# byronknoll/cmix

Hardware: AMD Instinct MI355X
Metric: input bytes/s on enwik8 at 1 GPU; compressed-size parity vs CPU ref (higher is better)
Workload: dtype f32

## Files before the change

### cmix_amd/csrc/cmx_api.hip

```cpp
#include <hip/hip_runtime.h>
#include <math.h>
#include <stdio.h>
#include <stdlib.h>
#include <string.h>
#include <stddef.h>
#include <string>
#include <map>
#include <mutex>
#include <vector>

#include "../../include/cmix_amd.h"
#include "mixnet_state.h"
#include "cmx_late.h"
#include "cmx_streams.h"
#include "cmx_verify.h"

extern "C" __global__ void cmx_mixnet_kernel(MixState*, const float*, const uint32_t*,
                                             const uint8_t*, const float*, int, float*, float*, int);
extern "C" __global__ void cmx_mixnet_spec_kernel(MixState*, SpecXfer*, const float*, const uint32_t*, const uint8_t*, const float*, int, float*,
                                                  float*, int);
extern "C" __global__ void cmx_mixnet_spec_jitter_kernel(MixState*, SpecXfer*, const float*, const uint32_t*, const uint8_t*, const float*, int, float*, float*, int);
extern "C" __global__ void cmx_mixnet_spec_late_kernel(MixState*, SpecXfer*, const float*, const uint32_t*, const float*, int, float*, float*, int, CmxLate);
extern "C" __global__ void cmx_mixnet_spec_verify_kernel(MixState*, SpecXfer*, const float*, const uint32_t*, const uint8_t*, const float*, int, float*, float*, int,
                                                         CmxVerify);
// ... 243 lines not shown
  ALLOC(map_keys, uint32_t, (size_t)CMX_MIXERS * CMX_MAP_SLOTS, true);
  ALLOC(map_vals, uint32_t, (size_t)CMX_MIXERS * CMX_MAP_SLOTS, true);
  ALLOC(s6, uint16_t, (size_t)CMX_SM6_VOL * 8, false);
  ALLOC(s7, uint16_t, (size_t)CMX_SM7_VOL * 8, false);
  ALLOC(x1, int, CMX_MIX1_VOL, false);
  ALLOC(x2, int, CMX_MIX2_VOL, false);
#undef ALLOC
  for (int i = 0; i <= CMX_MIXERS; ++i) S.max_steps[i] = 1;
  S.steps = 0;
  S.sse_j = 1;
  S.sse_pc = 0;
  S.sse_ffl = 0;
  for (int i = 0; i <= CMX_MIXERS; ++i) S.fwd_p[i] = 0.5f;
  h->d_state = (MixState*)dalloc(sizeof(MixState), false);
  if (!h->d_state) { set_err("hipMalloc failed for state"); cmx_mixnet_destroy(h); return nullptr; }
  hipMemcpy(h->d_state, &S, sizeof S, hipMemcpyHostToDevice);
  hipLaunchKernelGGL(cmx_sse_init_kernel, dim3(2048), dim3(256), 0, 0, h->d_state);
  h->d_sync_probs = (float*)dalloc(CMX_IN0 * 4, true);
  h->d_sync_sel = (uint32_t*)dalloc(CMX_MIXERS * 4, true);
  h->d_sync_bit = (uint8_t*)dalloc(16, true);
  h->d_sync_p = (float*)dalloc(16, true);
  if (hipFuncSetAttribute((const void*)cmx_mixnet_kernel, hipFuncAttributeMaxDynamicSharedMemorySize,
                          (int)kLdsBytes) != hipSuccess) {
    set_err("hipFuncSetAttribute(MaxDynamicSharedMemorySize) failed");
    cmx_mixnet_destroy(h);
    return nullptr;
  }
  h->d_xfer = (SpecXfer*)dalloc(sizeof(SpecXfer), true);
  bool attr_ok = true;
  for (const void* k : {(const void*)cmx_mixnet_spec_kernel, (const void*)cmx_mixnet_spec_jitter_kernel, (const void*)cmx_mixnet_spec_late_kernel,
                        (const void*)cmx_mixnet_spec_verify_kernel})
    attr_ok = attr_ok && hipFuncSetAttribute(k, hipFuncAttributeMaxDynamicSharedMemorySize, CMX_SPEC_LDS_BYTES) == hipSuccess;
  if (!h->d_xfer || !attr_ok) {
    set_err("cmx_mixnet_create: hand-off area / kernel attribute (spec kernel) failed");
    cmx_mixnet_destroy(h);
    return nullptr;
  }
  { const char* v = getenv("CMX_MIXNET_DBG"); h->dbg = v ? atoi(v) : 0; }
  { const char* v = getenv("CMX_MIXNET_JITTER"); h->jitter = v ? atoi(v) & 15 : 0; }
  { const char* v = getenv("CMX_MIXNET_ROTATE"); h->rotate = v && v[0] == '1'; }
  { const char* v = getenv("CMX_MIXNET_XCD"); h->xcd = v ? atoi(v) : CMX_MIXNET_XCD_DEFAULT; if (h->xcd > 7) h->xcd = -1; }
  hipEventCreate(&h->ev0);
  hipEventCreate(&h->ev1);
  for (int i = 0; i < CMX_PIPELINE_SLOTS; ++i) { hipEventCreateWithFlags(&h->ev_decay[i], hipEventDisableTiming); hipEventCreateWithFlags(&h->ev_kdone[i], hipEventDisableTiming); }
  hipError_t e = hipDeviceSynchronize();
  if (e != hipSuccess) { set_err(std::string("init: ") + hipGetErrorString(e)); cmx_mixnet_destroy(h); return nullptr; }
  return h;
}

static inline float decay_of(uint64_t steps) {
  return (float)(0.9 / pow(0.0000001 * steps + 0.8, 0.8));
}

static int ensure_decay(cmx_mixnet_t* h, size_t nbits) {
  const int fail_value = 1;
  if (nbits <= h->decay_cap) return 0;
  size_t cap = nbits < 4096 ? 4096 : nbits;
  if (h->h_decay) hipHostFree(h->h_decay);
  h->h_decay = nullptr;
  for (int i = 0; i < CMX_PIPELINE_SLOTS; ++i) {
    if (h->decay_used[i]) { (void)hipEventSynchronize(h->ev_decay[i]); (void)hipEventSynchronize(h->ev_kdone[i]); }
    h->decay_used[i] = false;
  }
  HIP_OK(hipHostMalloc((void**)&h->h_decay, (size_t)CMX_PIPELINE_SLOTS * cap * 4, hipHostMallocDefault));
  void* p = nullptr;
  HIP_OK(hipMalloc(&p, (size_t)CMX_PIPELINE_SLOTS * cap * 4));
  h->allocs.push_back(p);
  h->d_decay = (float*)p;
  h->decay_cap = cap;
  return 0;
}

int cmx_mixnet_spec_stats(cmx_mixnet_t* h, uint64_t out[5]) {
  const int fail_value = 1;
  if (!h || !out) { set_err("cmx_mixnet_spec_stats: bad argument"); return 1; }
  HIP_OK(hipSetDevice(h->device));
  HIP_OK(hipDeviceSynchronize());
  unsigned long long st[8];
  HIP_OK(hipMemcpy(st, (char*)h->d_xfer + offsetof(SpecXfer, stat), sizeof st, hipMemcpyDeviceToHost));
  for (int i = 0; i < 5; ++i) out[i] = st[i];
  return 0;
}

static bool g_cumask_applied = false;
static bool cumask_wanted() {
  static const char* const xe = getenv("CMX_MIXNET_XCD");
  static const bool w = getenv("CMX_CUMASK") != nullptr && xe && atoi(xe) >= 0 && atoi(xe) < 8 && getenv("CMX_PIPELINE_STREAMS") == nullptr;
  return w;
}
namespace {
std::mutex g_q_mu;
std::map<hipStream_t, int> g_q_dev;
int g_q_held[64];
}
int cmx_make_stream(hipStream_t* st, int which) {
  *st = nullptr;
  int dev = 0, cus = 0;
  if (hipGetDevice(&dev) != hipSuccess || hipDeviceGetAttribute(&cus, hipDeviceAttributeMultiprocessorCount, dev) != hipSuccess || cus <= 0 || cus > 32 * 32) {
    set_err("cmx_make_stream: no device"); return 1;
  }
  std::lock_guard<std::mutex> g(g_q_mu);
  int& held = g_q_held[dev & 63];
  if (held + 1 > CMX_MAX_HW_QUEUES) {
    set_err("cmx_make_stream: this process already holds " + std::to_string(held) + " dedicated hardware queues on device " + std::to_string(dev) + ", the limit is " +
            std::to_string(CMX_MAX_HW_QUEUES) + " (an engine takes 13, 14 when it decodes; CMX_PIPELINE_STREAMS=2 or 1 takes 8 or 6)");
    return 1;
  }
  const int words = (cus + 31) / 32;
  std::vector<uint32_t> full(words, 0u);
  for (int cu = 0; cu < cus; ++cu) full[cu / 32] |= 1u << (cu % 32);
  hipError_t e = hipErrorUnknown;
  if (cumask_wanted() && which != 2) {
    static const int x = atoi(getenv("CMX_MIXNET_XCD"));
    std::vector<uint32_t> m(words, 0u);
    for (int cu = 0; cu < cus; ++cu) if (((cu & 7) == x) == (which == 1)) m[cu / 32] |= 1u << (cu % 32);
    e = hipExtStreamCreateWithCUMask(st, (uint32_t)words, m.data());
    if (e == hipSuccess) { if (which == 1) g_cumask_applied = true; }
    else (void)hipGetLastError();
  }
  if (e != hipSuccess) e = hipExtStreamCreateWithCUMask(st, (uint32_t)words, full.data());
  if (e != hipSuccess) { *st = nullptr; set_err(std::string("cmx_make_stream: hipExtStreamCreateWithCUMask: ") + hipGetErrorString(e)); return 1; }
  g_q_dev[*st] = dev;
  ++held;
  return 0;
}
void cmx_destroy_stream(hipStream_t st) {
  if (!st) return;
  {
    std::lock_guard<std::mutex> g(g_q_mu);
    auto it = g_q_dev.find(st);
    if (it != g_q_dev.end()) { --g_q_held[it->second & 63]; g_q_dev.erase(it); }
  }
  (void)hipStreamDestroy(st);
}
int cmx_hw_queues(int device) {
  std::lock_guard<std::mutex> g(g_q_mu);
  return g_q_held[device & 63];
}

__global__ void cmx_overlap_probe_kernel(unsigned* cnt, unsigned* seen, int i, unsigned n, unsigned long long ticks) {
  if (threadIdx.x != 0) return;
  __hip_atomic_fetch_add(cnt, 1u, __ATOMIC_RELAXED, __HIP_MEMORY_SCOPE_AGENT);
  const unsigned long long t0 = wall_clock64();
  unsigned c = __hip_atomic_load(cnt, __ATOMIC_RELAXED, __HIP_MEMORY_SCOPE_AGENT);
  while (c < n && wall_clock64() - t0 < ticks) { __builtin_amdgcn_s_sleep(8); c = __hip_atomic_load(cnt, __ATOMIC_RELAXED, __HIP_MEMORY_SCOPE_AGENT); }
  __hip_atomic_store(seen + i, c, __ATOMIC_RELAXED, __HIP_MEMORY_SCOPE_AGENT);
}
int cmx_overlap_probe(const hipStream_t* st, int n, int* distinct) {
  std::vector<hipStream_t> q;
  for (int i = 0; i < n; ++i) {
    if (!st[i]) continue;
    bool dup = false;
    for (hipStream_t s : q) dup = dup || s == st[i];
    if (!dup) q.push_back(st[i]);
  }
  if (distinct) *distinct = (int)q.size();
  if (q.empty()) return 0;
  int dev = 0, khz = 0;
  if (hipGetDevice(&dev) != hipSuccess || hipDeviceGetAttribute(&khz, hipDeviceAttributeWallClockRate, dev) != hipSuccess || khz <= 0) { set_err("cmx_overlap_probe: no device"); return -1; }
  const int m = (int)q.size();
  unsigned* d = nullptr;
  if (hipMalloc((void**)&d, (size_t)(1 + m) * 4) != hipSuccess) { set_err("cmx_overlap_probe: hipMalloc failed"); return -1; }
  bool ok = hipMemsetAsync(d, 0, (size_t)(1 + m) * 4, q[0]) == hipSuccess && hipStreamSynchronize(q[0]) == hipSuccess;
  const unsigned long long ticks = 50ull * (unsigned long long)khz;
  for (int i = 0; ok && i < m; ++i) {
    hipLaunchKernelGGL(cmx_overlap_probe_kernel, dim3(1), dim3(64), 0, q[i], d, d + 1, i, (unsigned)m, ticks);
// ... 429 lines not shown
```

### cmix_amd/csrc/mixnet_chunk.hip

```cpp
#include "mixnet_dev.h"
#include "cmx_late.h"
#include "cmx_verify.h"

namespace {

constexpr int SEG = 548;
constexpr unsigned SPIN_LIMIT = 1u << 27;

struct Ctl {
  int staged[2];
  int consumed;
  int u_epoch;
  int scout_epoch;
  int tail_in;
  int tail_done;
  int abort;
  int b_in, b_done;
  int bit_epoch;
  unsigned late_lo, late_hi;
};

struct BitRec {
  uint32_t rowidx[48];
  uint32_t changed[32];
// ... 46 lines not shown
}

__device__ __forceinline__ unsigned long long wave_sum_u64(unsigned long long v) {
#pragma unroll
  for (int o = 32; o > 0; o >>= 1) v += __shfl_xor(v, o, 64);
  return v;
}
__device__ __forceinline__ void verify_flag(const CmxVerify& V, unsigned long long key) {
  atomicAdd(&V.hdr->launch_count, 1ull);
  atomicMax(&V.hdr->launch_first, ~key);
}

typedef __attribute__((address_space(3))) int lds_int;
__device__ __forceinline__ int lds_poll(const int* p) {
  int v;
  asm volatile("ds_read_b32 %0, %1\n\ts_waitcnt lgkmcnt(0)" : "=v"(v) : "v"((const lds_int*)p) : "memory");
  return v;
}
__device__ __forceinline__ void lds_publish_store(int* p, int v) {
  asm volatile("s_waitcnt lgkmcnt(0)\n\tds_write_b32 %0, %1" :: "v"((lds_int*)p), "v"(v) : "memory");
}
__device__ __forceinline__ void touch_line(gptr<const float> g, unsigned lds_dst) {
  unsigned keep;
  const unsigned dst = __builtin_amdgcn_readfirstlane(lds_dst);
  asm volatile("s_mov_b32 %0, m0\n\ts_mov_b32 m0, %2\n\ts_nop 0\n\tglobal_load_lds_dword %1, off\n\ts_mov_b32 m0, %0"
               : "=&s"(keep) : "v"(g), "s"(dst) : "memory");
}
__device__ __forceinline__ void st_rel(int* p, int v) { lds_publish_store(p, v); }
__device__ __forceinline__ CmxLateBox* ctl_box(Ctl* ctl) {
  const unsigned lo = (unsigned)lds_poll((const int*)&ctl->late_lo), hi = (unsigned)lds_poll((const int*)&ctl->late_hi);
  return reinterpret_cast<CmxLateBox*>(((unsigned long long)hi << 32) | lo);
}
__device__ __forceinline__ bool late_expired(CmxLateBox* B, unsigned long long& t0) {
  if (late_ld(&B->abort) || late_ld(&B->fail)) return true;
  const unsigned long long now = wall_clock64();
  if (!t0) { t0 = now; return false; }
  if (now - t0 > late_timeout_ticks(B)) { late_st(&B->fail, 1u); return true; }
  return false;
}
template <bool LATE = false> __device__ __forceinline__ bool wait_ge(Ctl* ctl, const int* p, int target, bool sleepy) {
  unsigned spins = 0;
  unsigned long long t0 = 0;
  while (lds_poll(p) < target) {
    if (sleepy) __builtin_amdgcn_s_sleep(2);
    if ((++spins & 1023u) == 0) {
      bool out;
      if (LATE) { CmxLateBox* const B = ctl_box(ctl); out = B ? late_expired(B, t0) : spins > SPIN_LIMIT; }
      else out = spins > SPIN_LIMIT;
      if (lds_poll(&ctl->abort) || out) {
        lds_publish_store(&ctl->abort, 1);
        return false;
      }
    }
  }
  return true;
}

__device__ __forceinline__ float bcast_lane(float v, int j) {
  return __int_as_float(__builtin_amdgcn_readlane(__float_as_int(v), j));
}

__device__ __forceinline__ float clamp_med3(float x, float mn, float mx) { return __builtin_amdgcn_fmed3f(x, mn, mx); }
__device__ __forceinline__ float clamp_out(float x, float mn, float mx) {
  const float lo = x < mn ? mn : x;
  return x > mx ? mx : lo;
}

__device__ __forceinline__ float4 f4sub_mul(float4 w, float u, float4 x) {
  w.x = fsub(w.x, fmul(u, x.x));
  w.y = fsub(w.y, fmul(u, x.y));
  w.z = fsub(w.z, fmul(u, x.z));
  w.w = fsub(w.w, fmul(u, x.w));
  return w;
}
__device__ __forceinline__ float4 f4scale(float4 w, float c) {
  w.x = fmul(w.x, c); w.y = fmul(w.y, c); w.z = fmul(w.z, c); w.w = fmul(w.w, c);
  return w;
}
__device__ __forceinline__ float add4(float p, float4 v) {
  p = fadd(p, v.x); p = fadd(p, v.y); p = fadd(p, v.z); p = fadd(p, v.w);
  return p;
}

template <int NB> __device__ __forceinline__ float chain_seg_n(const float* rowp, int n, float p) {
  const float4* row = reinterpret_cast<const float4*>(__builtin_assume_aligned(rowp, 16));
  float4 a[8], b[8];
#pragma unroll
  for (int i = 0; i < 8; ++i) a[i] = row[i];
#pragma unroll 1
  for (int bi = 0; bi < NB; bi += 2) {
    __builtin_amdgcn_sched_barrier(0);
#pragma unroll
    for (int i = 0; i < 8; ++i) b[i] = row[(bi + 1) * 8 + i];
    __builtin_amdgcn_sched_barrier(0);
#pragma unroll
    for (int i = 0; i < 8; ++i) p = add4(p, a[i]);
    __builtin_amdgcn_sched_barrier(0);
#pragma unroll
    for (int i = 0; i < 8; ++i) a[i] = row[(bi + 2) * 8 + i];
    __builtin_amdgcn_sched_barrier(0);
#pragma unroll
    for (int i = 0; i < 8; ++i) p = add4(p, b[i]);
  }
  __builtin_amdgcn_sched_barrier(0);
  const int rem4 = (n >> 2) - NB * 8;
#pragma unroll
  for (int i = 0; i < 7; ++i)
    if (i < rem4) p = add4(p, a[i]);
  if (n & 2) {
    p = fadd(p, a[7].x);
    p = fadd(p, a[7].y);
  }
  return p;
}

struct U16x8 { unsigned w0, w1, w2, w3; };
__device__ __forceinline__ U16x8 load_cell(const uint16_t* p) {
  typedef unsigned v4u __attribute__((ext_vector_type(4)));
  v4u v = *(gptr<const v4u>)as_global(p);
  U16x8 r; r.w0 = v.x; r.w1 = v.y; r.w2 = v.z; r.w3 = v.w;
  return r;
}
__device__ __forceinline__ void store_cell_async(uint16_t* p, const U16x8& c) {
  typedef unsigned v4u __attribute__((ext_vector_type(4)));
  v4u o = {c.w0, c.w1, c.w2, c.w3};
  asm volatile("global_store_dwordx4 %0, %1, off\n\ts_nop 1" :: "v"(as_global(p)), "v"(o) : "memory");
}
__device__ __forceinline__ int cell_get(const U16x8& c, int i) {
  unsigned w = i < 2 ? c.w0 : i < 4 ? c.w1 : i < 6 ? c.w2 : c.w3;
  return (int)((i & 1) ? (w >> 16) : (w & 0xffffu));
}
__device__ __forceinline__ void cell_set(U16x8& c, int i, int v) {
  const unsigned m = (i & 1) ? 0x0000ffffu : 0xffff0000u, x = ((unsigned)v & 0xffffu) << ((i & 1) * 16);
  const int q = i >> 1;
  c.w0 = q == 0 ? (c.w0 & m) | x : c.w0;
  c.w1 = q == 1 ? (c.w1 & m) | x : c.w1;
  c.w2 = q == 2 ? (c.w2 & m) | x : c.w2;
  c.w3 = q == 3 ? (c.w3 & m) | x : c.w3;
}
__device__ __forceinline__ unsigned bcast_u(unsigned v) { return (unsigned)__builtin_amdgcn_readlane((int)v, 0); }

struct SseInterp {
  int freq, sw, P;
  __device__ __forceinline__ int pred(const U16x8& c, int iP) {
    freq = (6 * iP) >> 15;
    sw = (6 * iP) & 32767;
    int f = (((32768 - sw) * cell_get(c, freq) + sw * cell_get(c, freq + 1)) >> 15) - 8192;
    if (f <= 0) f = 1;
    if (f >= 32768) f = 32767;
    P = f;
    return f;
  }
  __device__ __forceinline__ void update(U16x8& c, int bit, int wr0) {
    P = (P * (32768 - wr0)) >> 15;
    if (bit == 0) P += wr0;
    const int c0 = cell_get(c, freq), c1 = cell_get(c, freq + 1);
    const int dC = c0 - c1;
    const int sw_dC = (sw * dC + 32767) >> 15;
    cell_set(c, freq, (uint16_t)(P + sw_dC + 8192));
    cell_set(c, freq + 1, (uint16_t)(P - (dC - sw_dC) + 8192));
  }
};

template <bool LATE, bool JIT = false, bool VER = false> __device__ void tail_a_role(MixState* S, const Lds& L, const float* decay1, int nbits, float* mix_out, int lane, bool prof_on,
                                                                     const CmxVerify& V) {
  uint64_t tprev = __builtin_readcyclecounter();
  uint64_t pacc[6] = {0, 0, 0, 0, 0, 0};
#define TPROF(k) do { if (prof_on) { uint64_t now_ = __builtin_readcyclecounter(); pacc[k - 6] += now_ - tprev; tprev = now_; } } while (0)
  const int k = lane;
  const bool is1 = k < CMX_MIX1;
  const int kk = is1 ? k : 0;
  const float smin = S->stretch_min, smax = S->stretch_max;
  const float cdec = 1.0f - 3.0e-6f;
  const float lr1 = S->lr[CMX_MIX0 + kk];
  const gptr<float> rows1 = as_global(S->rows1);
  const gptr<uint64_t> row_steps = as_global(S->row_steps);
  uint64_t mx1 = S->max_steps[CMX_MIX0 + kk], rs1 = 0;
  float* const w1 = L.w1 + kk * 68;
  uint32_t cur_row = 0xffffffffu;
  gptr<float> row1 = rows1;
  gptr<uint64_t> rsp1 = row_steps;
  auto store_row1 = [&]() {
#pragma unroll
    for (int i = 0; i < 13; ++i) gstore4_async(row1 + 4 * i, *reinterpret_cast<const float4*>(w1 + 4 * i));
    asm volatile("global_store_dwordx2 %0, %1, off\n\ts_nop 0" :: "v"(rsp1), "v"(rs1) : "memory");
  };
  unsigned long long vdec = 0;
  asm volatile("s_waitcnt lgkmcnt(0)" ::: "memory");
  for (int t = 0; t < nbits; ++t) {
    TPROF(11);
    jitter_stall<JIT>(L.jit, t, 1);
    if (!wait_ge<LATE>(L.ctl, &L.ctl->scout_epoch, t + 1, true)) return;
    const BitRec* rec = L.rec + (t % L.rr);
    const uint32_t newrow = rec->rowidx[CMX_MIX0 + kk];
// ... 249 lines not shown
    if (k < CMX_IN2) {
      float v = fsub(w2[k], fmul(u2, in2[k]));
      if (df2) v = fmul(v, cdec);
      w2[k] = v;
    }
    asm volatile("s_waitcnt lgkmcnt(0)" ::: "memory");
    __builtin_amdgcn_wave_barrier();
    st_rel(&L.ctl->b_done, t + 1);
    TPROF(2);
    if constexpr (VER) {
      if ((t + 1) % CMX_VERIFY_BLOCK == 0 || t + 1 == nbits) {
        if (lane == 0) as_global(V.rec)[(size_t)(t / CMX_VERIFY_BLOCK) * CMX_VERIFY_REC + CMX_VR_DECAY + 2] = vdec;
        vdec = 0;
      }
    }
  }
  if (prof_on && lane == 0) {
#pragma unroll
    for (int i = 0; i < 3; ++i) S->prof[13 + i] += pacc[i];
  }
#undef TPROF
  if (nbits > 0) {
    asm volatile("s_waitcnt lgkmcnt(0)" ::: "memory");
    __builtin_amdgcn_wave_barrier();
    if (k < 16 && cur_row2 != 0xffffffffu)
      gstore4(rows2 + (size_t)cur_row2 * CMX_ROW2_STRIDE + 4 * k, *reinterpret_cast<const float4*>(w2 + 4 * k));
    if (k == 0) {
      if (cur_row2 != 0xffffffffu) rsteps2[cur_row2] = rs2;
      S->max_steps[CMX_MIXERS - 1] = mx2;
      S->sse_j = sj; S->sse_pc = spc; S->sse_ffl = sffl;
      S->steps = S->steps + steps_done;
    }
  }
}


struct HelperLds {
  float prod[4][SEG];
  double segsum[4];
  float res[4];
  int sum_epoch[4];
  int res_epoch[4];
  int abort;
  int pad_;
};

__device__ __forceinline__ unsigned long long ld_u64(const unsigned long long* p) { return __hip_atomic_load(p, __ATOMIC_RELAXED, __HIP_MEMORY_SCOPE_AGENT); }
__device__ __forceinline__ void st_u64(unsigned long long* p, unsigned long long v) { __hip_atomic_store(p, v, __ATOMIC_RELAXED, __HIP_MEMORY_SCOPE_AGENT); }
__device__ __forceinline__ unsigned ld_u32(const unsigned* p) { return __hip_atomic_load(p, __ATOMIC_RELAXED, __HIP_MEMORY_SCOPE_AGENT); }
__device__ __forceinline__ float ld_f32(const float* p) { return __hip_atomic_load(p, __ATOMIC_RELAXED, __HIP_MEMORY_SCOPE_AGENT); }
constexpr unsigned SPEC_SPIN = 1u << 24;

__device__ __forceinline__ int f2ord(float f) { int b = __float_as_int(f); return b ^ ((b >> 31) & 0x7fffffff); }
__device__ __forceinline__ float ord2f(int o) { return __int_as_float(o ^ ((o >> 31) & 0x7fffffff)); }

template <int CTRL> __device__ __forceinline__ double dpp_f64(double v) {
  const int lo = __builtin_amdgcn_update_dpp(0, __double2loint(v), CTRL, 0xf, 0xf, false);
  const int hi = __builtin_amdgcn_update_dpp(0, __double2hiint(v), CTRL, 0xf, 0xf, false);
  return __hiloint2double(hi, lo);
}
__device__ __forceinline__ double readlane_f64(double v, int l) {
  return __hiloint2double(__builtin_amdgcn_readlane(__double2hiint(v), l), __builtin_amdgcn_readlane(__double2loint(v), l));
}
__device__ __forceinline__ double wave_sum_f64(double v) {
  v += dpp_f64<0xB1>(v);
  v += dpp_f64<0x4E>(v);
  v += dpp_f64<0x124>(v);
  v += dpp_f64<0x128>(v);
  return (readlane_f64(v, 0) + readlane_f64(v, 16)) + (readlane_f64(v, 32) + readlane_f64(v, 48));
}

template <bool LATE, bool JIT = false, bool VER = false> __device__ void helper_role(MixState* S, SpecXfer* X, HelperLds* H, int nbits, int m, int w, int lane, bool tol, CmxLateBox* LB,
                                                                  bool local, int jit, const CmxLate& late, const float* probs, const CmxVerify& V) {
  const gptr<float> rows0 = as_global(S->rows0);
  const gptr<const float> lut = as_global(S->logit_lut);
  constexpr int NW = 4, SEGN = 2048 / NW, KS = SEGN / 64, LASTW = NW - 1;
  const int base = SEGN * w;
  const int nseg = w == LASTW ? CMX_IN0 - SEGN * LASTW : SEGN;
  const bool tailk = w == LASTW && lane < 30;
  const float cdec = 1.0f - 3.0e-6f;
  float W[KS + 1], Wn[KS + 1], xc[KS + 1], xp[KS + 1];
#pragma unroll
  for (int k = 0; k < KS + 1; ++k) { W[k] = 0.0f; Wn[k] = 0.0f; xc[k] = 0.0f; xp[k] = 0.0f; }
  unsigned long long n_spec = 0, n_hit = 0, n_miss = 0;
  uint32_t cur_base = 0;
  bool f_chg = false; uint32_t f_base = 0;
  auto failed = [&]() { return lds_poll(&H->abort) != 0; };
  unsigned long long late_t0 = 0;
  auto spun_out = [&](unsigned spins) { return LATE ? late_expired(LB, late_t0) : spins > SPEC_SPIN; };
  auto give_up = [&]() { lds_publish_store(&H->abort, 1); __hip_atomic_store(&X->fail, 1u, __ATOMIC_RELAXED, __HIP_MEMORY_SCOPE_AGENT); };
  auto seg_digest = [&](const float* v, uint32_t segt) -> unsigned long long {
    unsigned long long d = 0;
#pragma unroll
    for (int k = 0; k < KS; ++k) d += cmx_vmix(CMX_VC_SEGMENT, segt, (uint32_t)(base + 64 * k + lane), __float_as_uint(v[k]));
    if (tailk) d += cmx_vmix(CMX_VC_SEGMENT, segt, (uint32_t)(base + SEGN + lane), __float_as_uint(v[KS]));
    return wave_sum_u64(d);
  };
  unsigned long long vring = 0;
  float Wev[KS + 1];
  uint32_t ev_segt = 0; bool ev_pend = false;
  auto seg_store = [&]() {
    if constexpr (VER) {
      if (!ev_pend) return;
      ev_pend = false;
      const unsigned long long d = seg_digest(Wev, ev_segt);
      if (lane == 0) as_global(V.seg)[(size_t)ev_segt * CMX_VERIFY_SEGS + w] = d;
    }
  };
  auto fetch = [&](int t) -> bool {
    unsigned spins = 0;
    const unsigned* const ep = LATE && m != CMX_AUX ? &X->sel_epoch : &X->scout_epoch;
    while (ld_u32(ep) < (unsigned)(t + 1)) {
      __builtin_amdgcn_s_sleep(1);
      if ((++spins & 1023u) == 0 && (spun_out(spins) || failed() || ld_u32(&X->fail))) { give_up(); return false; }
    }
    late_t0 = 0;
    const int slot = t % CMX_SPEC_RING;
    f_chg = ld_u32(&X->changed[slot][m]) != 0;
    if (f_chg) {
      const uint32_t nb = ((uint32_t)m * CMX_ROWS_PER_MIXER + ld_u32(&X->rowidx[slot][m])) * CMX_ROW0_STRIDE + (uint32_t)base;
      f_base = nb;
#pragma unroll
      for (int k = 0; k < KS; ++k) Wn[k] = rows0[nb + 64 * k + lane];
      Wn[KS] = tailk ? rows0[nb + SEGN + lane] : 0.0f;
      if constexpr (VER) {
        const uint32_t segt = (nb - (uint32_t)base) / CMX_ROW0_STRIDE;
        const unsigned long long want = as_global(V.seg)[(size_t)segt * CMX_VERIFY_SEGS + w];
        const unsigned long long got = seg_digest(Wn, segt);
        if (lane == 0 && want != 0 && want != got)
          verify_flag(V, cmx_vkey((uint32_t)t / CMX_VERIFY_BLOCK, CMX_VC_SEGMENT, (uint32_t)m, segt - (uint32_t)m * CMX_ROWS_PER_MIXER, (uint32_t)w));
      }
    }
    if (LATE) {
      const unsigned need = w == 0 ? (1u << LC_CTX) | (1u << LC_BM0) | (1u << LC_FX) | (1u << LC_P8) : w == LASTW ? (1u << LC_P8) | (1u << LC_CTX) | (1u << LC_BM1) | (1u << LC_BM2) : (1u << LC_P8);
      bool ok = true;
      if (lane <= LC_P8 && ((need >> lane) & 1u)) ok = late_wait_cnt(late, lane, (uint32_t)(t + 1));
      if (__ballot(!ok)) { give_up(); return false; }
      const float* row = probs + (size_t)t * CMX_IN0 + base;
      float pv[KS + 1];
#pragma unroll
      for (int k = 0; k < KS; ++k) pv[k] = __hip_atomic_load(row + 64 * k + lane, __ATOMIC_RELAXED, __HIP_MEMORY_SCOPE_AGENT);
      pv[KS] = tailk ? __hip_atomic_load(row + SEGN + lane, __ATOMIC_RELAXED, __HIP_MEMORY_SCOPE_AGENT) : 0.5f;
#pragma unroll
      for (int k = 0; k < KS + 1; ++k) {
        float p = pv[k];
        if (p < 1.0e-4f) p = 1.0e-4f;
        else if (p > 1 - 1.0e-4f) p = 1 - 1.0e-4f;
        int idx = (int)(p * 100001.0f);
        if (idx >= 100001) idx = 100000;
        else if (idx < 0) idx = 0;
        xc[k] = lut[idx];
      }
      if (!tailk) xc[KS] = 0.0f;
    } else {
      const float* gx = X->xs[slot] + base;
#pragma unroll
      for (int k = 0; k < KS; ++k) xc[k] = ld_f32(gx + 64 * k + lane);
      xc[KS] = tailk ? ld_f32(gx + SEGN + lane) : 0.0f;
      if constexpr (VER) {
#pragma unroll
        for (int k = 0; k < KS; ++k) vring += cmx_vmix(CMX_VC_RING_WRITTEN, (uint32_t)t, (uint32_t)(base + 64 * k + lane), __float_as_uint(xc[k]));
        if (tailk) vring += cmx_vmix(CMX_VC_RING_WRITTEN, (uint32_t)t, (uint32_t)(base + SEGN + lane), __float_as_uint(xc[KS]));
        if ((t + 1) % CMX_VERIFY_BLOCK == 0 || t + 1 == nbits) {
          const unsigned long long v = wave_sum_u64(vring);
          if (lane == 0) as_global(V.rec)[(size_t)(t / CMX_VERIFY_BLOCK) * CMX_VERIFY_REC + CMX_VR_RINGR + 4 * m + w] = v;
          vring = 0;
        }
      }
    }
    return true;
  };
  auto apply_u = [&](int tu) -> bool {
    unsigned long long v;
    unsigned spins = 0;
    while ((unsigned)((v = ld_u64(&X->u[m])) >> 33) != (unsigned)tu) {
      if ((++spins & 1023u) == 0 && (spun_out(spins) || failed() || ld_u32(&X->fail))) { give_up(); return false; }
    }
    late_t0 = 0;
    const float u = __int_as_float((int)(unsigned)v);
    const bool df = ((v >> 32) & 1ull) != 0;
#pragma unroll
    for (int k = 0; k < KS + 1; ++k) {
      W[k] = fsub(W[k], fmul(u, xp[k]));
      if (df) W[k] = fmul(W[k], cdec);
    }
    return true;
  };
  if (nbits > 0 && !fetch(0)) return;
  for (int t = 0; t <= nbits; ++t) {
    const bool live = t < nbits;
    jitter_stall<JIT>(jit, t, 16 + 4 * m + w);
    if (t > 0 && !LATE) { if (!apply_u(t)) return; }
    const bool chg = !live || f_chg;
    if (chg) {
      if (t > 0) {
#pragma unroll
        for (int k = 0; k < KS; ++k) rows0[cur_base + 64 * k + lane] = W[k];
        if (tailk) rows0[cur_base + SEGN + lane] = W[KS];
        if constexpr (VER) {
#pragma unroll
          for (int k = 0; k < KS + 1; ++k) Wev[k] = W[k];
          ev_segt = (cur_base - (uint32_t)base) / CMX_ROW0_STRIDE; ev_pend = true;
        }
      }
      if (live) {
        cur_base = f_base;
#pragma unroll
        for (int k = 0; k < KS + 1; ++k) W[k] = Wn[k];
      }
    }
    if (!live) { seg_store(); break; }
    float* pr = H->prod[w];
    double ds = 0.0;
#pragma unroll
    for (int k = 0; k < KS; ++k) { const float p = fmul(xc[k], W[k]); pr[64 * k + lane] = p; ds += (double)p; }
    if (w == LASTW) { const float p = tailk ? fmul(xc[KS], W[KS]) : 0.0f; if (lane < 36) pr[SEGN + lane] = p; ds += (double)p; }
#pragma unroll
    for (int k = 0; k < KS + 1; ++k) xp[k] = xc[k];
    if (tol) {
      ds = wave_sum_f64(ds);
      if (w < LASTW) {
        if (lane == 0) H->segsum[w] = ds;
        asm volatile("s_waitcnt lgkmcnt(0)" ::: "memory");
        if (lane == 0) lds_publish_store(&H->sum_epoch[w], t + 1);
      } else {
        double tot = 0.0;
        for (int q = 0; q < LASTW; ++q) {
          unsigned spins = 0;
          while (lds_poll(&H->sum_epoch[q]) < t + 1)
            if ((++spins & 1023u) == 0 && (spins > SPEC_SPIN || failed())) { give_up(); return; }
          tot += H->segsum[q];
        }
        tot += ds;
        if (lane == 0) st_u64(&X->sum[m], ((unsigned long long)(unsigned)(t + 1) << 32) | (unsigned)__float_as_int((float)tot));
      }
      seg_store();
      if (t + 1 < nbits && !fetch(t + 1)) return;
      continue;
    }
    if (w < LASTW) {
      ds = wave_sum_f64(ds);
      if (lane == 0) H->segsum[w] = ds;
      asm volatile("s_waitcnt lgkmcnt(0)" ::: "memory");
      if (lane == 0) lds_publish_store(&H->sum_epoch[w], t + 1);
    }
    asm volatile("s_waitcnt lgkmcnt(0)" ::: "memory");
    __builtin_amdgcn_wave_barrier();
    float start = 0.0f;
    if (w > 0) {
      double est = 0.0;
      for (int q = 0; q < w; ++q) {
        unsigned spins = 0;
        while (lds_poll(&H->sum_epoch[q]) < t + 1)
          if ((++spins & 1023u) == 0 && (spins > SPEC_SPIN || failed())) { give_up(); return; }
        est += H->segsum[q];
      }
      start = ord2f(f2ord((float)est) + lane - 32);
    }
    float r = chain_seg_n<16>(pr, nseg, start);
    if (w > 0) {
      unsigned spins = 0;
      while (lds_poll(&H->res_epoch[w - 1]) < t + 1)
        if ((++spins & 1023u) == 0 && (spins > SPEC_SPIN || failed())) { give_up(); return; }
      const float s = H->res[w - 1];
      const unsigned long long hit = __ballot(__float_as_int(start) == __float_as_int(s));
      ++n_spec;
      if (hit) {
        r = __int_as_float(__builtin_amdgcn_readlane(__float_as_int(r), (int)__builtin_amdgcn_readfirstlane(__ffsll((long long)hit) - 1)));
        ++n_hit;
      } else {
        r = chain_seg_n<16>(pr, nseg, s);
        ++n_miss;
      }
    }
    if (w < LASTW) {
      if (lane == 0) H->res[w] = r;
      asm volatile("s_waitcnt lgkmcnt(0)" ::: "memory");
      if (lane == 0) lds_publish_store(&H->res_epoch[w], t + 1);
    } else if (lane == 0) {
      const unsigned long long word = ((unsigned long long)(unsigned)(t + 1) << 32) | (unsigned)__float_as_int(r);
      if (local) asm volatile("global_store_dwordx2 %0, %1, off" :: "v"(&X->sum[m]), "v"(word) : "memory");
      else st_u64(&X->sum[m], word);
    }
    jitter_stall<JIT>(jit, t, 144 + 4 * m + w);
    if (LATE && !apply_u(t + 1)) return;
    seg_store();
    if (t + 1 < nbits && !fetch(t + 1)) return;
  }
  asm volatile("s_waitcnt vmcnt(0)" ::: "memory");
  if (lane == 0 && w > 0) {
    atomicAdd(&X->stat[0], n_spec); atomicAdd(&X->stat[1], n_hit); atomicAdd(&X->stat[1 + w], n_miss);
  }
}

template <bool LATE, bool JIT = false, bool VER = false> __device__ void stretch_role(MixState* S, const Lds& L, SpecXfer* X, const float* probs, const uint8_t* bits, int nbits, int sw,
                                                                      int lane, const CmxVerify& V) {
  const gptr<const float> lut = as_global(S->logit_lut);
  const gptr<const float> gprobs = as_global(probs);
  const float smin = S->stretch_min, smax = S->stretch_max;
  unsigned long long vrow = 0, vbit = 0, vring = 0;
  for (int t = sw; t < nbits; t += 4) {
    jitter_stall<JIT>(L.jit, t, 4 + sw);
    if (t >= L.lead && !wait_ge<LATE>(L.ctl, &L.ctl->consumed, 4 * (t - L.lead) + 1, true)) return;
    if (t >= L.rr && !wait_ge<LATE>(L.ctl, &L.ctl->tail_done, t - L.rr + 1, true)) return;
    BitRec* rec = L.rec + (t % L.rr);
    const gptr<const float> pr = gprobs + (size_t)t * CMX_IN0;
    if (LATE) {
      bool ok = true;
      if (lane <= LC_P8) ok = late_wait_cnt(L.late, lane, (uint32_t)(t + 1));
      if (__ballot(!ok)) { lds_publish_store(&L.ctl->abort, 1); return; }
      if (lane == 0) late_stamp(L.late, 2);
    }
    float pv[33];
    if (LATE) {
#pragma unroll
      for (int r = 0; r < 33; ++r) {
        int i = r * 64 + lane;
        pv[r] = i < CMX_IN0 ? __hip_atomic_load(probs + (size_t)t * CMX_IN0 + i, __ATOMIC_RELAXED, __HIP_MEMORY_SCOPE_AGENT) : 0.5f;
      }
    } else {
#pragma unroll
      for (int r = 0; r < 33; ++r) {
        int i = r * 64 + lane;
        pv[r] = i < CMX_IN0 ? pr[i] : 0.5f;
      }
    }
    if constexpr (VER) {
#pragma unroll
      for (int r = 0; r < 33; ++r)
        if (r * 64 + lane < CMX_IN0) vrow += cmx_vmix(CMX_VC_ROW, (uint32_t)t, (uint32_t)(r * 64 + lane), __float_as_uint(pv[r]));
    }
    const int bitv = LATE ? 0 : (int)bits[t];
    if constexpr (VER) { if (lane == 0) vbit += cmx_vmix(CMX_VC_BIT, (uint32_t)t, 0, (uint32_t)bitv); }
    const float lstm_raw = bcast_lane(pv[32], 29);
#pragma unroll
    for (int r = 0; r < 33; ++r) {
      float p = pv[r];
      if (p < 1.0e-4f) p = 1.0e-4f;
      else if (p > 1 - 1.0e-4f) p = 1 - 1.0e-4f;
      int idx = (int)(p * 100001.0f);
      if (idx >= 100001) idx = 100000;
      else if (idx < 0) idx = 0;
      pv[r] = lut[idx];
    }
    if (!LATE) {
      float* gx = X->xs[t % CMX_SPEC_RING];
#pragma unroll
      for (int r = 0; r < 33; ++r) {
        int i = r * 64 + lane;
        if constexpr (VER) {
          if (i < CMX_IN0) {
            vring += cmx_vmix(CMX_VC_RING_WRITTEN, (uint32_t)t, (uint32_t)i, __float_as_uint(pv[r]));
            const float sv = (t == V.pert_bit && i == V.pert_index) ? __uint_as_float(__float_as_uint(pv[r]) ^ V.pert_mask) : pv[r];
            __hip_atomic_store(gx + i, sv, __ATOMIC_RELAXED, __HIP_MEMORY_SCOPE_AGENT);
          }
        } else {
          if (i < CMX_IN0) __hip_atomic_store(gx + i, pv[r], __ATOMIC_RELAXED, __HIP_MEMORY_SCOPE_AGENT);
        }
      }
    }
    const float ax0 = bcast_lane(pv[6], 49), ax1 = bcast_lane(pv[31], 40), ax2 = bcast_lane(pv[32], 29);
    if (lane < 3) {
      float v = lane == 0 ? ax0 : lane == 1 ? ax1 : ax2;
      if (v > smax) v = smax;
      else if (v < smin) v = smin;
      rec->aux3[lane] = v;
    } else if (lane == 3) {
      float avg = 0;
      avg = fadd(avg, cmx_logistic(ax0));
      avg = fadd(avg, cmx_logistic(ax1));
      avg = fadd(avg, cmx_logistic(ax2));
      avg = avg / 3.0f;
      rec->auxkey = (uint32_t)(unsigned long long)(avg * 15);
      rec->lstm_p = lstm_raw;
// ... 484 lines not shown
```

### cmix_amd/engine.py

```python
import ctypes as C
import os

import numpy as np

HERE = os.path.dirname(os.path.abspath(__file__))
LIB_PATH = os.path.join(HERE, "lib", "libcmixamd.so")

N_INPUTS, N_MIXERS = 2078, 47
PIPELINE_SLOTS = 8


class CmxError(RuntimeError):
    pass


_lib = None


def lib():
    global _lib
    if _lib is None:
        if not os.path.exists(LIB_PATH):
            raise CmxError(f"{LIB_PATH} is missing: run `python -m cmix_amd.build` "
                           "(there is no non-HIP fallback)")
# ... 454 lines not shown
            raise CmxError(last_error())
        return _state_diff(out)

    def debug_state_xor(self, region, mixer, row, index, xor_mask):
        if lib().cmx_mixnet_debug_state_xor(self.h, _region(region), _u64(mixer), _u64(row), _u64(index), int(xor_mask)):
            raise CmxError(last_error())

    def close(self):
        if getattr(self, "h", None):
            lib().cmx_mixnet_destroy(self.h)
            self.h = None

    def __del__(self):
        try:
            self.close()
        except Exception:
            pass

    def run(self, probs, sel, bits, p_out=None, mix_out=None, stream=None):
        import torch
        T = int(bits.numel())
        assert probs.is_cuda and sel.is_cuda and bits.is_cuda
        assert probs.dtype == torch.float32 and probs.is_contiguous() and probs.numel() == T * N_INPUTS
        assert sel.dtype == torch.int32 and sel.is_contiguous() and sel.numel() == T * N_MIXERS
        assert bits.dtype == torch.uint8 and bits.is_contiguous()
        if p_out is None:
            p_out = torch.empty(T, dtype=torch.float32, device=probs.device)
        if stream is None:
            stream = torch.cuda.current_stream(probs.device).cuda_stream
        rc = lib().cmx_mixnet_run(self.h, probs.data_ptr(), sel.data_ptr(), bits.data_ptr(), T,
                                  p_out.data_ptr(), mix_out.data_ptr() if mix_out is not None else None,
                                  C.c_void_p(stream))
        if rc:
            raise CmxError(last_error())
        return p_out

    def predict(self, probs, sel):
        probs = np.ascontiguousarray(probs, np.float32)
        sel = np.ascontiguousarray(sel, np.uint32)
        assert probs.size == N_INPUTS and sel.size == N_MIXERS
        p = lib().cmx_mixnet_predict(self.h, probs.ctypes.data, sel.ctypes.data)
        if p < 0:
            raise CmxError(last_error())
        return np.float32(p)

    def perceive(self, bit):
        if lib().cmx_mixnet_perceive(self.h, int(bit)):
            raise CmxError(last_error())

    def sync(self):
        if lib().cmx_mixnet_sync(self.h):
            raise CmxError(last_error())

    def bits_done(self):
        v = C.c_uint64(0)
        if lib().cmx_mixnet_bits_done(self.h, C.byref(v)):
            raise CmxError(last_error())
        return v.value

    def profile(self, enable=True):
        out = (C.c_uint64 * 16)()
        if lib().cmx_mixnet_profile(self.h, int(enable), out):
            raise CmxError(last_error())
        return list(out)

    def last_kernel_ms(self):
        v = C.c_float(0)
        if lib().cmx_mixnet_last_kernel_ms(self.h, C.byref(v)):
            raise CmxError(last_error())
        return v.value

    def debug_set_steps(self, steps):
        lib().cmx_mixnet_debug_set_steps.argtypes = [C.c_void_p, C.c_uint64]
        if lib().cmx_mixnet_debug_set_steps(self.h, int(steps)):
            raise CmxError(last_error())

    def spec_stats(self):
        out = (C.c_uint64 * 5)()
        if lib().cmx_mixnet_spec_stats(self.h, out):
            raise CmxError(last_error())
        v = list(out)
        return {"segments": v[0], "hits": v[1], "reruns": v[2:5], "hit_rate": (v[1] / v[0]) if v[0] else None}


class Lstm:
    SKIP_RAND = 31

    def __init__(self, vocab, device=0, skip_rand=SKIP_RAND):
        vocab = np.ascontiguousarray(vocab, np.uint8)
        assert vocab.size == 256
        self.h = lib().cmx_lstm_create(vocab.ctypes.data, skip_rand, device)
        if not self.h:
            raise CmxError(last_error())
        self.V = lib().cmx_lstm_vocab_size(self.h)

    def set_tolerance(self, on=True):
        if lib().cmx_lstm_set_tolerance(self.h, 1 if on else 0):
            raise CmxError(last_error())

    def close(self):
        if getattr(self, "h", None):
            lib().cmx_lstm_destroy(self.h)
            self.h = None

    def __del__(self):
        try:
            self.close()
        except Exception:
            pass

    def run(self, in_probs, data, want_bits=True, stream=None, layer0=None, out=None):
        import torch
        N = int(data.numel())
        assert in_probs.is_cuda and in_probs.dtype == torch.float32 and in_probs.is_contiguous()
        assert in_probs.numel() == N * 256 and data.dtype == torch.uint8 and data.is_contiguous()
        if out is None:
            out = torch.empty((N, 256), dtype=torch.float32, device=in_probs.device)
        bp, bp_ptr, stride = None, None, 1
        if layer0 is not None:
            assert layer0.dtype == torch.float32 and layer0.is_contiguous() and layer0.shape == (8 * N, N_INPUTS)
            bp_ptr, stride = layer0.data_ptr() + 4 * (N_INPUTS - 1), N_INPUTS
        elif want_bits:
            bp = torch.empty((N, 8), dtype=torch.float32, device=in_probs.device)
            bp_ptr = bp.data_ptr()
        bx = torch.empty((N, 8), dtype=torch.int32, device=in_probs.device) if bp_ptr else None
        if stream is None:
            stream = torch.cuda.current_stream(in_probs.device).cuda_stream
        rc = lib().cmx_lstm_run(self.h, in_probs.data_ptr(), data.data_ptr(), N, out.data_ptr(),
                                bp_ptr, stride, bx.data_ptr() if bx is not None else None, C.c_void_p(stream))
        if rc:
            raise CmxError(last_error())
        return out, bp, bx

    def gate_weights(self, layer, gate):
        n = lib().cmx_lstm_gate_rowlen(self.h, layer)
        out = np.empty((200, n), np.float32)
        if lib().cmx_lstm_get_gate_weights(self.h, layer, gate, out.ctypes.data):
            raise CmxError("cmx_lstm_get_gate_weights failed")
        return out


SMALL_COLS = [0, 1, 2] + list(range(2025, 2076))


class CtxModels:

    def __init__(self, vocab, device=0, compact=False):
        vocab = np.ascontiguousarray(vocab, np.uint8)
        assert vocab.size == 256
        self.compact = bool(compact)
        self.h = (lib().cmx_ctxmodels_create_compact if self.compact else lib().cmx_ctxmodels_create)(vocab.ctypes.data, device)
        if not self.h:
            raise CmxError(last_error())

    def state_diff(self, other):
        out = (C.c_uint64 * 16)()
        if lib().cmx_ctxmodels_state_diff(self.h, other.h, out):
            raise CmxError(last_error())
        return _ctx_state_diff(out)

    def debug_state_xor(self, region, lane, index, xor_mask):
        if lib().cmx_ctxmodels_debug_state_xor(self.h, _ctx_region(region), _u64(lane), int(index), int(xor_mask)):
            raise CmxError(last_error())

    def close(self):
        if getattr(self, "h", None):
# ... 619 lines not shown
```

### include/cmix_amd.h

```cpp
#ifndef CMIX_AMD_H
#define CMIX_AMD_H

#include <stddef.h>
#include <stdint.h>

#ifdef __cplusplus
extern "C" {
#endif

#define CMX_N_INPUTS 2078
#define CMX_N_MIXERS 47
#define CMX_N_MIX0 26
#define CMX_N_MIX1 20
#define CMX_AUX_MIXER 12

const char* cmx_last_error(void);
int cmx_device_count(void);
const char* cmx_version(void);
void* cmx_device_alloc(int device, size_t bytes);
void cmx_device_free(int device, void* p);
void* cmx_host_alloc(size_t bytes);
void cmx_host_free(void* p);
int cmx_copy_to_host(int device, void* dst, const void* d_src, size_t bytes);

typedef struct cmx_engine cmx_t;
cmx_t* cmx_create(const uint8_t vocab[256], const char* dict_path, int device);
float cmx_predict(cmx_t*);
int cmx_perceive(cmx_t*, int bit);
int cmx_pretrain(cmx_t*, int bit);
int cmx_decode_stream(cmx_t*, const uint8_t* code, size_t code_len, uint8_t* out, size_t nbytes);
int cmx_set_model_outputs(cmx_t*, const float cols_3_to_2024[2022]);
int cmx_get_lstm_hint(cmx_t*, int* lstmpr, int* lstmex);
const float* cmx_debug_last_row(cmx_t*);
int cmx_stage_input(cmx_t*, const uint8_t* bytes, size_t n);
int cmx_mode(cmx_t*, int* chunks_in_flight);
int cmx_set_verify(cmx_t*, int on);
int cmx_verify_report(cmx_t*, uint64_t out[8]);
int cmx_set_shadow(cmx_t*, int k);
int cmx_shadow_report(cmx_t*, uint64_t out[8]);
int cmx_set_shadow_repair(cmx_t*, int max_repairs);
int cmx_shadow_repairs(cmx_t*, uint64_t out[], size_t cap);
int cmx_debug_shadow_xor(cmx_t*, uint64_t after_chunk, int instance, int region, uint64_t mixer, uint64_t row, uint64_t index, uint32_t xor_mask);
int cmx_set_ctx_shadow(cmx_t*, int k);
int cmx_ctx_shadow_report(cmx_t*, uint64_t out[8]);
int cmx_debug_ctx_shadow_xor(cmx_t*, uint64_t after_chunk, int instance, int region, uint64_t lane, uint64_t index, uint32_t xor_mask);
void cmx_destroy(cmx_t*);

typedef struct cmx_mixnet cmx_mixnet_t;
cmx_mixnet_t* cmx_mixnet_create(int device);
void cmx_mixnet_destroy(cmx_mixnet_t*);

int cmx_mixnet_set_tolerance(cmx_mixnet_t*, int on);
const int* cmx_mixnet_error_flag(cmx_mixnet_t*);
int cmx_mixnet_mode(cmx_mixnet_t*);
int cmx_mixnet_set_upload_stream(cmx_mixnet_t*, void* stream);
int cmx_mixnet_run(cmx_mixnet_t*, const float* d_probs, const uint32_t* d_sel,
                   const uint8_t* d_bits, size_t nbits, float* d_p_out, float* d_mix_out,
                   void* stream);

float cmx_mixnet_predict(cmx_mixnet_t*, const float* probs2078, const uint32_t* sel47);
int cmx_mixnet_perceive(cmx_mixnet_t*, int bit);

int cmx_mixnet_predict_async(cmx_mixnet_t*, const float* d_probs2078, const uint32_t* d_sel47, float* d_p, void* stream);
int cmx_mixnet_perceive_async(cmx_mixnet_t*, int bit, void* stream);

int cmx_mixnet_sync(cmx_mixnet_t*);

int cmx_mixnet_bits_done(const cmx_mixnet_t*, uint64_t* out);
int cmx_mixnet_profile(cmx_mixnet_t*, int enable, uint64_t* out16);
int cmx_mixnet_last_kernel_ms(cmx_mixnet_t*, float* ms);
int cmx_mixnet_spec_stats(cmx_mixnet_t*, uint64_t out[5]);
int cmx_mixnet_debug_set_steps(cmx_mixnet_t*, uint64_t steps);
int cmx_mixnet_set_verify(cmx_mixnet_t*, int on);
int cmx_mixnet_verify_on(cmx_mixnet_t*);
int cmx_mixnet_verify_report(cmx_mixnet_t*, uint64_t out[8]);
const unsigned long long* cmx_mixnet_verify_record(cmx_mixnet_t*);
int cmx_mixnet_debug_verify_perturb(cmx_mixnet_t*, int cls, uint64_t bit, uint64_t index, uint32_t xor_mask);

typedef struct cmx_vote cmx_vote_t;
cmx_vote_t* cmx_vote_create(int device, int n);
void cmx_vote_destroy(cmx_vote_t*);
int cmx_vote_run(cmx_vote_t*, const float* const* d_p, const float* const* d_mix, size_t nbits, uint64_t stream_bit0, const uint32_t* d_sel,
                 const uint8_t* d_bits, void* stream);
int cmx_vote_report(cmx_vote_t*, uint64_t out[8]);
const unsigned long long* cmx_vote_record(cmx_vote_t*);
int cmx_vote_values(cmx_vote_t*, uint32_t words[144], uint32_t sel[47], uint32_t* bit);
int cmx_vote_last(cmx_vote_t*, uint64_t out[4]);
int cmx_mixnet_state_diff(cmx_mixnet_t* a, cmx_mixnet_t* b, uint64_t out[20]);
int cmx_mixnet_state_repair(cmx_mixnet_t* dst, cmx_mixnet_t* src, uint64_t out[20]);
int cmx_mixnet_debug_state_xor(cmx_mixnet_t*, int region, uint64_t mixer, uint64_t row, uint64_t index, uint32_t xor_mask);

typedef struct cmx_lstm cmx_lstm_t;
cmx_lstm_t* cmx_lstm_create(const uint8_t vocab[256], int skip_rand, int device);
void cmx_lstm_destroy(cmx_lstm_t*);
int cmx_lstm_vocab_size(const cmx_lstm_t*);
int cmx_lstm_run(cmx_lstm_t*, const float* d_in_probs, const uint8_t* d_bytes, size_t nbytes,
                 float* d_out_probs, float* d_bit_p, size_t bit_p_stride, int* d_bit_ex, void* stream);
int cmx_bytemodel_bits_run(int device, const float* d_dist0, const float* d_dist_rest,
                           const uint8_t* d_bytes, size_t nbytes, float* d_bit_p, size_t bit_p_stride,
                           int* d_bit_ex, void* stream);
int cmx_bytemodel_bit_run(int device, const float* d_dist, const uint8_t* d_byte, int k, float* d_bit_p,
                          size_t bit_p_stride, int* d_bit_ex, float* d_p_copy, void* stream);
int cmx_lstm_get_gate_weights(cmx_lstm_t*, int layer, int gate, float* out_host);
int cmx_lstm_gate_rowlen(const cmx_lstm_t*, int layer);
int cmx_lstm_failed(cmx_lstm_t*);
int cmx_lstm_set_tolerance(cmx_lstm_t*, int on);
const unsigned* cmx_lstm_fail_flag(cmx_lstm_t*);
int cmx_glibc_rand_selftest(uint32_t seed, int n, int* out);

typedef struct cmx_ctxmodels cmx_ctxmodels_t;
cmx_ctxmodels_t* cmx_ctxmodels_create(const uint8_t vocab[256], int device);
void cmx_ctxmodels_destroy(cmx_ctxmodels_t*);
int cmx_ctxmodels_run(cmx_ctxmodels_t*, const uint8_t* d_bytes, size_t nbytes, float* d_probs, size_t pstride,
                      uint32_t* d_sel, void* stream);
int cmx_ctxmodels_peek(cmx_ctxmodels_t*, const uint8_t* d_byte, int bit_index ,
                       float* d_probs8, size_t probs_stride, uint32_t* d_sel8, void* stream);
int cmx_ctxmodels_pretrain(cmx_ctxmodels_t*, const uint8_t* d_bytes, size_t nbytes, void* stream);
int cmx_ctxmodels_debug_slow_bytes(cmx_ctxmodels_t*, uint64_t out2[2]);
int cmx_ctxmodels_debug_set_history(cmx_ctxmodels_t*, uint64_t pos, const uint8_t* tail, uint64_t n);
int cmx_ctxmodels_sync(cmx_ctxmodels_t*);
int cmx_ctxmodels_get_manager(cmx_ctxmodels_t*, uint64_t* regs25, uint64_t* ctx54, uint64_t* bitctx8);
#define CMX_CTX_COMPACT_STRIDE 64
cmx_ctxmodels_t* cmx_ctxmodels_create_compact(const uint8_t vocab[256], int device);
#define CMX_CTXVOTE_COLS 101
typedef struct cmx_ctxvote cmx_ctxvote_t;
cmx_ctxvote_t* cmx_ctxvote_create(int device, int n);
void cmx_ctxvote_destroy(cmx_ctxvote_t*);
int cmx_ctxvote_run(cmx_ctxvote_t*, const float* const* d_probs, const size_t* pstride, const int* compact, const uint32_t* const* d_sel, size_t nbits,
                    uint64_t stream_bit0, const uint8_t* d_bits, void* stream);
int cmx_ctxvote_report(cmx_ctxvote_t*, uint64_t out[8]);
const unsigned long long* cmx_ctxvote_record(cmx_ctxvote_t*);
int cmx_ctxvote_values(cmx_ctxvote_t*, uint32_t words[3 * CMX_CTXVOTE_COLS], uint32_t* bit);
int cmx_ctxvote_last(cmx_ctxvote_t*, uint64_t out[4]);
int cmx_ctxmodels_state_diff(cmx_ctxmodels_t* a, cmx_ctxmodels_t* b, uint64_t out[16]);
int cmx_ctxmodels_debug_state_xor(cmx_ctxmodels_t*, int region, uint64_t lane, uint64_t index, uint32_t xor_mask);
int cmx_ctxmodels_debug_layout(uint64_t out[5]);

typedef struct cmx_fxcm cmx_fxcm_t;
cmx_fxcm_t* cmx_fxcm_create(const char* dictionary_path, int device);
void cmx_fxcm_destroy(cmx_fxcm_t*);
int cmx_fxcm_run(cmx_fxcm_t*, const uint8_t* bytes, const uint8_t* d_bytes, size_t nbytes, const int16_t* d_lstmpr, const uint8_t* d_lstmex,
                 float* d_probs, size_t pstride, void* stream);
int cmx_fxcm_sync(cmx_fxcm_t*);
int cmx_fxcm_failed(cmx_fxcm_t*);
const unsigned* cmx_fxcm_fail_flag(cmx_fxcm_t*);
int cmx_fxcm_set_upload_stream(cmx_fxcm_t*, void* stream);
int cmx_fxcm_profile(cmx_fxcm_t*, unsigned long long out128[128]);

typedef struct cmx_encoder cmx_encoder_t;
typedef struct cmx_decoder cmx_decoder_t;
cmx_encoder_t* cmx_encoder_create(void);
void cmx_encoder_destroy(cmx_encoder_t*);
int cmx_encoder_encode_bits(cmx_encoder_t*, const float* p, const uint8_t* bits, size_t nbits);
int cmx_encoder_encode_bytes(cmx_encoder_t*, const float* p , const uint8_t* bytes, size_t nbytes);
// ... 131 lines not shown
```

Before: 17780.

## Speculate mid-segment sum on miss to split serial chain rerun in halves

When the speculative segment sum misses, the helper now estimates the midpoint partial sum with a double-precision wave reduction, has each lane try a neighbouring float candidate for the second half in parallel, and checks which candidate matches the exact serial first-half sum computed on lane 0. On a mid hit, the serial rerun covers only half the segment; otherwise the second half is rerun serially after the first. This is meant to shorten the serial fallback latency on misses, at the cost of an extra reduction and counters, with new stats exposed through an API call.

```diff
diff --git a/cmix_amd/csrc/cmx_api.hip b/cmix_amd/csrc/cmx_api.hip
--- a/cmix_amd/csrc/cmx_api.hip
+++ b/cmix_amd/csrc/cmx_api.hip
@@ -349,6 +349,17 @@
   return 0;
 }
 
+int cmx_mixnet_spec_rerun_stats(cmx_mixnet_t* h, uint64_t out[2]) {
+  const int fail_value = 1;
+  if (!h || !out) { set_err("cmx_mixnet_spec_rerun_stats: bad argument"); return 1; }
+  HIP_OK(hipSetDevice(h->device));
+  HIP_OK(hipDeviceSynchronize());
+  unsigned long long st[8];
+  HIP_OK(hipMemcpy(st, (char*)h->d_xfer + offsetof(SpecXfer, stat), sizeof st, hipMemcpyDeviceToHost));
+  out[0] = st[5]; out[1] = st[6];
+  return 0;
+}
+
 static bool g_cumask_applied = false;
 static bool cumask_wanted() {
   static const char* const xe = getenv("CMX_MIXNET_XCD");
diff --git a/cmix_amd/csrc/mixnet_chunk.hip b/cmix_amd/csrc/mixnet_chunk.hip
--- a/cmix_amd/csrc/mixnet_chunk.hip
+++ b/cmix_amd/csrc/mixnet_chunk.hip
@@ -152,7 +152,7 @@
   return p;
 }
 
-template <int NB> __device__ __forceinline__ float chain_seg_n(const float* rowp, int n, float p) {
+template <int NB> __device__ __forceinline__ float chain_seg_n(const float* rowp, int n, float p, bool rem_on = true) {
   const float4* row = reinterpret_cast<const float4*>(__builtin_assume_aligned(rowp, 16));
   float4 a[8], b[8];
 #pragma unroll
@@ -174,12 +174,14 @@
   }
   __builtin_amdgcn_sched_barrier(0);
   const int rem4 = (n >> 2) - NB * 8;
-#pragma unroll
-  for (int i = 0; i < 7; ++i)
-    if (i < rem4) p = add4(p, a[i]);
-  if (n & 2) {
-    p = fadd(p, a[7].x);
-    p = fadd(p, a[7].y);
+  if (rem_on) {
+#pragma unroll
+    for (int i = 0; i < 7; ++i)
+      if (i < rem4) p = add4(p, a[i]);
+    if (n & 2) {
+      p = fadd(p, a[7].x);
+      p = fadd(p, a[7].y);
+    }
   }
   return p;
 }
@@ -595,7 +597,7 @@
   float W[KS + 1], Wn[KS + 1], xc[KS + 1], xp[KS + 1];
 #pragma unroll
   for (int k = 0; k < KS + 1; ++k) { W[k] = 0.0f; Wn[k] = 0.0f; xc[k] = 0.0f; xp[k] = 0.0f; }
-  unsigned long long n_spec = 0, n_hit = 0, n_miss = 0;
+  unsigned long long n_spec = 0, n_hit = 0, n_miss = 0, n_mid = 0, n_ser = 0;
   uint32_t cur_base = 0;
   bool f_chg = false; uint32_t f_base = 0;
   auto failed = [&]() { return lds_poll(&H->abort) != 0; };
@@ -724,9 +726,9 @@
     }
     if (!live) { seg_store(); break; }
     float* pr = H->prod[w];
-    double ds = 0.0;
-#pragma unroll
-    for (int k = 0; k < KS; ++k) { const float p = fmul(xc[k], W[k]); pr[64 * k + lane] = p; ds += (double)p; }
+    double ds = 0.0, dh = 0.0;
+#pragma unroll
+    for (int k = 0; k < KS; ++k) { const float p = fmul(xc[k], W[k]); pr[64 * k + lane] = p; ds += (double)p; if (k == KS / 2 - 1) dh = ds; }
     if (w == LASTW) { const float p = tailk ? fmul(xc[KS], W[KS]) : 0.0f; if (lane < 36) pr[SEGN + lane] = p; ds += (double)p; }
 #pragma unroll
     for (int k = 0; k < KS + 1; ++k) xp[k] = xc[k];
@@ -782,7 +784,18 @@
         r = __int_as_float(__builtin_amdgcn_readlane(__float_as_int(r), (int)__builtin_amdgcn_readfirstlane(__ffsll((long long)hit) - 1)));
         ++n_hit;
       } else {
-        r = chain_seg_n<16>(pr, nseg, s);
+        const double me = (double)s + wave_sum_f64(dh);
+        const float cand = ord2f(f2ord((float)me) + lane - 32);
+        const float h = chain_seg_n<8>(pr + (lane ? SEGN / 2 : 0), nseg - SEGN / 2, lane ? cand : s, lane != 0);
+        const float mid = bcast_lane(h, 0);
+        const unsigned long long mhit = __ballot(lane != 0 && __float_as_int(cand) == __float_as_int(mid));
+        if (mhit) {
+          r = __int_as_float(__builtin_amdgcn_readlane(__float_as_int(h), (int)__builtin_amdgcn_readfirstlane(__ffsll((long long)mhit) - 1)));
+          ++n_mid;
+        } else {
+          r = chain_seg_n<8>(pr + SEGN / 2, nseg - SEGN / 2, mid);
+          ++n_ser;
+        }
         ++n_miss;
       }
     }
@@ -803,6 +816,7 @@
   asm volatile("s_waitcnt vmcnt(0)" ::: "memory");
   if (lane == 0 && w > 0) {
     atomicAdd(&X->stat[0], n_spec); atomicAdd(&X->stat[1], n_hit); atomicAdd(&X->stat[1 + w], n_miss);
+    atomicAdd(&X->stat[5], n_mid); atomicAdd(&X->stat[6], n_ser);
   }
 }
 
diff --git a/cmix_amd/engine.py b/cmix_amd/engine.py
--- a/cmix_amd/engine.py
+++ b/cmix_amd/engine.py
@@ -560,6 +560,13 @@
         v = list(out)
         return {"segments": v[0], "hits": v[1], "reruns": v[2:5], "hit_rate": (v[1] / v[0]) if v[0] else None}
 
+    def spec_rerun_stats(self):
+        out = (C.c_uint64 * 2)()
+        lib().cmx_mixnet_spec_rerun_stats.argtypes = [C.c_void_p, C.c_void_p]
+        if lib().cmx_mixnet_spec_rerun_stats(self.h, out):
+            raise CmxError(last_error())
+        return {"mid_hits": int(out[0]), "serial_halves": int(out[1])}
+
 
 class Lstm:
     SKIP_RAND = 31
diff --git a/include/cmix_amd.h b/include/cmix_amd.h
--- a/include/cmix_amd.h
+++ b/include/cmix_amd.h
@@ -70,6 +70,7 @@
 int cmx_mixnet_profile(cmx_mixnet_t*, int enable, uint64_t* out16);
 int cmx_mixnet_last_kernel_ms(cmx_mixnet_t*, float* ms);
 int cmx_mixnet_spec_stats(cmx_mixnet_t*, uint64_t out[5]);
+int cmx_mixnet_spec_rerun_stats(cmx_mixnet_t*, uint64_t out[2]);
 int cmx_mixnet_debug_set_steps(cmx_mixnet_t*, uint64_t steps);
 int cmx_mixnet_set_verify(cmx_mixnet_t*, int on);
 int cmx_mixnet_verify_on(cmx_mixnet_t*);
```

Result: faster. 18600, median of 6 (+4.7%).
